# InternRobotics/InternNav

Measured on AMD Instinct MI355X. Metric: policy steps/sec/node, higher is better.
Workload: dtype bf16

## Files before the change

include/internnav_amd.h:

```cpp
#ifndef INTERNNAV_AMD_H
#define INTERNNAV_AMD_H

#include <stddef.h>
#include <stdint.h>

#ifdef __cplusplus
extern "C" {
#endif

#define INA_ABI_VERSION 8

#define INA_ACT_NONE_C 0
#define INA_ACT_GELU_ERF_C 1
#define INA_ACT_GELU_TANH_C 2
#define INA_ACT_RELU_C 3
#define INA_ACT_SILU_C 4
#define INA_ACT_MISH_C 5
#define INA_BF16 0
#define INA_F32 1

int ina_abi_version(void);
const char* ina_last_error(void);
int ina_device_check(char* name, int n);
int ina_struct_size(int k);
int ina_set_workspace_slot(int slot);
int ina_workspace_retired(void);
int ina_prof_enable(int on);
int ina_prof_read(int kind, double* ms_total, int64_t* launches, double* flops, double* bytes);
int ina_prof_read_sub(int kind, int sub, double* ms_total, int64_t* launches, double* flops, double* bytes);

typedef struct ina_gemm_args {
    const void* A;
    const void* W;
    void* C;
    const float* bias;
    const float* colscale;
    const float* rowscale;
    const void* R;
    int32_t M, N, K;
    int32_t lda, ldw, ldc, ldr;
    int32_t act;
    int32_t out_dtype;
    int32_t res_dtype;
    int32_t glu;
    int32_t rowscale_div;
    int32_t batch;
    int64_t strideA, strideW, strideC, strideR;
    int32_t force_cfg;
    int32_t group_m;
    const float* norm_gamma;
    float norm_eps;
    int32_t a_dtype;
    float* seg_stats;
    float seg_eps;
    int32_t _pad_seg;
    const void* Wp;
} ina_gemm_args;
int ina_gemm_bf16(const ina_gemm_args* args, void* stream);
int ina_gemm_w8(const ina_gemm_args* args, const void* W8, const int8_t* wexp, void* stream);
int ina_gemm_preshuffle(const void* W, void* Wp, int32_t N, int32_t K, int64_t ldw, void* stream);
int ina_gemm_select(const ina_gemm_args* args, int* kernel);

typedef struct ina_attn_args {
    const void* Q;
    const void* K;
    const void* V;
    void* O;
    int64_t q_bs, q_rs, q_hs;
    int64_t k_bs, k_rs, k_hs;
    int64_t v_bs, v_rs, v_hs;
    int64_t o_bs, o_rs, o_hs;
    int32_t B, H, Hkv;
    int32_t Lq, Lk;
    int32_t D;
    int32_t causal;
    int32_t kv_start;
    int32_t kv_bdiv;
    float scale;
    const int32_t* cu_q;
    const int32_t* cu_k;
    const float* head_gate;
    const int32_t* k_len;
    int32_t accumulate;
    uint32_t drop_seed;
    uint32_t drop_thresh;
    float drop_scale;
    int32_t kernel;
    int32_t _pad0;
    const uint32_t* drop_salt;
    const float* rope_cos;
    const float* rope_sin;
    const void* k_new;
    const void* v_new;
    int64_t kn_bs, kn_rs, kn_hs;
// ... 388 lines not shown
```

internnav_amd/_lib.py:

```python
from __future__ import annotations

import ctypes as C
from pathlib import Path

_HERE = Path(__file__).resolve().parent
LIB_PATH = _HERE / "libinternnav_amd.so"

c_void_p, c_int32, c_int64, c_float = C.c_void_p, C.c_int32, C.c_int64, C.c_float


class GemmArgs(C.Structure):
    _fields_ = [
        ("A", c_void_p), ("W", c_void_p), ("C", c_void_p),
        ("bias", c_void_p), ("colscale", c_void_p), ("rowscale", c_void_p), ("R", c_void_p),
        ("M", c_int32), ("N", c_int32), ("K", c_int32),
        ("lda", c_int32), ("ldw", c_int32), ("ldc", c_int32), ("ldr", c_int32),
        ("act", c_int32), ("out_dtype", c_int32), ("res_dtype", c_int32), ("glu", c_int32),
        ("rowscale_div", c_int32), ("batch", c_int32),
        ("strideA", c_int64), ("strideW", c_int64), ("strideC", c_int64), ("strideR", c_int64),
        ("force_cfg", c_int32), ("group_m", c_int32),
        ("norm_gamma", c_void_p), ("norm_eps", c_float), ("a_dtype", c_int32),
        ("seg_stats", c_void_p), ("seg_eps", c_float), ("_pad_seg", c_int32),
        ("Wp", c_void_p),
    ]


class AttnArgs(C.Structure):
    _fields_ = [
        ("Q", c_void_p), ("K", c_void_p), ("V", c_void_p), ("O", c_void_p),
        ("q_bs", c_int64), ("q_rs", c_int64), ("q_hs", c_int64),
        ("k_bs", c_int64), ("k_rs", c_int64), ("k_hs", c_int64),
        ("v_bs", c_int64), ("v_rs", c_int64), ("v_hs", c_int64),
        ("o_bs", c_int64), ("o_rs", c_int64), ("o_hs", c_int64),
        ("B", c_int32), ("H", c_int32), ("Hkv", c_int32),
        ("Lq", c_int32), ("Lk", c_int32), ("D", c_int32),
        ("causal", c_int32), ("kv_start", c_int32), ("kv_bdiv", c_int32),
        ("scale", c_float),
        ("cu_q", c_void_p), ("cu_k", c_void_p), ("head_gate", c_void_p), ("k_len", c_void_p),
        ("accumulate", c_int32), ("drop_seed", C.c_uint32), ("drop_thresh", C.c_uint32), ("drop_scale", c_float),
        ("kernel", c_int32), ("_pad0", c_int32), ("drop_salt", c_void_p),
        ("rope_cos", c_void_p), ("rope_sin", c_void_p), ("k_new", c_void_p), ("v_new", c_void_p),
        ("kn_bs", c_int64), ("kn_rs", c_int64), ("kn_hs", c_int64),
    ]


class RowMap(C.Structure):
    _fields_ = [("seg_len", c_int32), ("seg_stride", c_int32), ("off", c_int32), ("_pad", c_int32)]


class NormArgs(C.Structure):
    _fields_ = [
        ("X", c_void_p), ("Y", c_void_p), ("Y32", c_void_p),
        ("gamma", c_void_p), ("beta", c_void_p), ("mod_scale", c_void_p), ("gate", c_void_p), ("G", c_void_p), ("P", c_void_p),
        ("in_map", RowMap), ("out_map", RowMap),
        ("rows", c_int32), ("C", c_int32),
# ... 187 lines not shown
                ("lddp", c_int32), ("loss_scale", c_float)]


class AdamwArgs(C.Structure):
    _fields_ = [("p", c_void_p), ("g", c_void_p), ("m", c_void_p), ("v", c_void_p), ("p_bf16", c_void_p), ("sumsq_parts", c_void_p),
                ("norm_out", c_void_p), ("n", c_int64), ("n_parts", c_int32), ("zero_grad", c_int32),
                ("lr", c_float), ("beta1", c_float), ("beta2", c_float), ("eps", c_float), ("wd", c_float), ("bc1", c_float), ("bc2", c_float),
                ("max_norm", c_float), ("grad_scale", c_float), ("_pad", c_int32)]


class GemmDwArgs(C.Structure):
    _fields_ = [("DY", c_void_p), ("X", c_void_p), ("dW", c_void_p), ("db", c_void_p), ("partial", c_void_p), ("partial_elems", c_int64),
                ("rows", c_int32), ("N", c_int32), ("K", c_int32), ("dy_dt", c_int32), ("lddy", c_int32), ("ldx", c_int32), ("ldw", c_int32), ("splits", c_int32)]


class GemmNnArgs(C.Structure):
    _fields_ = [("X", c_void_p), ("W", c_void_p), ("partial", c_void_p), ("partial_elems", c_int64),
                ("M", c_int32), ("N", c_int32), ("K", c_int32), ("ldx", c_int32), ("ldw", c_int32), ("splits", c_int32)]


class AttnBwdArgs(C.Structure):
    _fields_ = [("f", AttnArgs), ("dO", c_void_p), ("dQ", c_void_p), ("dK", c_void_p), ("dV", c_void_p), ("lse", c_void_p), ("delta", c_void_p),
                ("dq_bs", c_int64), ("dq_rs", c_int64), ("dq_hs", c_int64), ("dkv_bs", c_int64), ("dkv_rs", c_int64), ("dkv_hs", c_int64),
                ("kv_row0", c_int32), ("nsplit", c_int32), ("part", c_void_p), ("dq32", c_void_p), ("stage", c_int32), ("_pad", c_int32)]


SYMBOLS = {
    "ina_abi_version": (C.c_int, []),
    "ina_last_error": (C.c_char_p, []),
    "ina_device_check": (C.c_int, [C.c_char_p, C.c_int]),
    "ina_gemm_bf16": (C.c_int, [C.POINTER(GemmArgs), c_void_p]),
    "ina_gemm_w8": (C.c_int, [C.POINTER(GemmArgs), c_void_p, c_void_p, c_void_p]),
    "ina_gemm_select": (C.c_int, [C.POINTER(GemmArgs), C.POINTER(C.c_int)]),
    "ina_gemm_preshuffle": (C.c_int, [c_void_p, c_void_p, c_int32, c_int32, c_int64, c_void_p]),
    "ina_attention_bf16": (C.c_int, [C.POINTER(AttnArgs), c_void_p]),
    "ina_norm_bf16": (C.c_int, [C.POINTER(NormArgs), c_void_p]),
    "ina_patchify": (C.c_int, [C.POINTER(PatchifyArgs), c_void_p]),
    "ina_embed3": (C.c_int, [C.POINTER(Embed3Args), c_void_p]),
    "ina_goal_slots": (C.c_int, [c_void_p, c_int32, c_int32, c_int32, c_int32, c_int32, c_void_p, c_int32, c_int32, c_void_p, c_void_p, c_void_p,
                                 c_void_p, c_int32, c_void_p, c_void_p, c_void_p, c_int32, c_void_p, c_void_p, c_void_p, c_int32, c_void_p,
                                 c_void_p, c_int32, c_int32, c_void_p]),
    "ina_kv_copy": (C.c_int, [c_int32, c_void_p, c_int32, c_void_p, c_int32, c_int64, c_int64, c_int64, c_void_p]),
    "ina_attention_prefix": (C.c_int, [c_void_p, c_int64, c_int64, c_int64, c_void_p, c_int64, c_int64, c_int64, c_void_p, c_void_p, c_int64, c_int64,
                                       c_int64, c_int32, c_void_p, c_void_p, c_int64, c_int64, c_int64, c_void_p, c_void_p, c_void_p, c_int32, c_int32,
                                       c_int32, c_int32, c_int32, c_int32, c_float, c_void_p]),
    "ina_memory_gather": (C.c_int, [c_void_p, c_int64, c_void_p, c_void_p, c_void_p, c_void_p, c_void_p, c_void_p, c_void_p, c_int32, c_int32, c_int32,
                                    c_int32, c_int32, c_int32, c_int32, c_void_p]),
    "ina_traj_actions": (C.c_int, [c_void_p, c_int32, c_int32, c_int32, c_int32, c_void_p, c_int32, c_void_p, c_void_p, c_int32, c_void_p]),
    "ina_head3": (C.c_int, [C.POINTER(Head3Args), c_void_p]),
    "ina_seqpool_head": (C.c_int, [C.POINTER(SeqpoolArgs), c_void_p]),
    "ina_select_traj": (C.c_int, [C.POINTER(SelectArgs), c_void_p]),
    "ina_pool_act": (C.c_int, [C.POINTER(PoolActArgs), c_void_p]),
    "ina_gather_rows": (C.c_int, [C.POINTER(GatherArgs), c_void_p]),
    "ina_rope_bf16": (C.c_int, [C.POINTER(RopeArgs), c_void_p]),
    "ina_mrope_table": (C.c_int, [C.POINTER(MropeTableArgs), c_void_p]),
    "ina_argmax_rows": (C.c_int, [C.POINTER(ArgmaxArgs), c_void_p]),
    "ina_token_seen_set": (C.c_int, [c_void_p, c_int32, c_void_p, c_int32, c_void_p, c_int32, c_int32, c_void_p]),
    "ina_argmax_penalty_rows": (C.c_int, [c_void_p, c_int32, c_int32, c_int32, c_void_p, c_int32, C.c_float, c_int32, c_void_p, c_void_p]),
    "ina_logprob_rows": (C.c_int, [c_void_p, c_int32, c_int32, c_int32, c_void_p, c_int32, C.c_float, c_int32, c_void_p, c_void_p, c_void_p, c_void_p,
                                   c_void_p]),
    "ina_dit_attention": (C.c_int, [C.POINTER(DitAttnArgs), c_void_p]),
    "ina_resize_u8": (C.c_int, [C.POINTER(ResizeU8Args), c_void_p]),
    "ina_qwen_patchify_u8": (C.c_int, [C.POINTER(QwenPatchifyArgs), c_void_p]),
    "ina_u8_lut": (C.c_int, [C.POINTER(U8LutArgs), c_void_p]),
    "ina_resize_f32": (C.c_int, [C.POINTER(ResizeF32Args), c_void_p]),
    "ina_dit_rowchain": (C.c_int, [C.POINTER(DitRowchainArgs), c_void_p]),
# ... 54 lines not shown
```

internnav_amd/csrc/abi.cpp:

```cpp
#include <stdarg.h>
#include <stdio.h>
#include <string.h>
#include <cmath>

#include "common.h"
#include "kernels.h"

static thread_local char g_err[1024] = "";

void ina_set_error(const char* fmt, ...) {
    va_list ap;
    va_start(ap, fmt);
    vsnprintf(g_err, sizeof(g_err), fmt, ap);
    va_end(ap);
}

#include <mutex>
#include <vector>
namespace {
struct ProfRec { int kind, sub; hipEvent_t a, b; double flops, bytes; };
thread_local int g_prof_sub = 0;
bool g_prof_on = false;
std::vector<ProfRec> g_prof;
std::mutex g_prof_mu;
// ... 167 lines not shown
}

int ina_traj_actions(void* traj, int32_t traj_dtype, int32_t B, int32_t S, int32_t T, int32_t* actions, int32_t max_actions, int32_t* count,
                     double* traj_out, int32_t scale_in_place, void* stream) {
    return ina_launch_traj_actions(traj, traj_dtype, B, S, T, actions, max_actions, count, traj_out, scale_in_place, reinterpret_cast<hipStream_t>(stream));
}

int ina_token_seen_set(uint32_t* seen, int32_t ld_words, const int32_t* ids, int32_t ld_ids, const int32_t* lens, int32_t rows, int32_t n, void* stream) {
    return ina_launch_token_seen_set(seen, ld_words, ids, ld_ids, lens, rows, n, reinterpret_cast<hipStream_t>(stream));
}

int ina_argmax_penalty_rows(const float* X, int32_t ldx, int32_t rows, int32_t n, uint32_t* seen, int32_t ld_words, float penalty, int32_t mark,
                            int32_t* out, void* stream) {
    return ina_launch_argmax_penalty(X, ldx, rows, n, seen, ld_words, penalty, mark, out, reinterpret_cast<hipStream_t>(stream));
}

int ina_logprob_rows(const float* X, int32_t ldx, int32_t rows, int32_t n, uint32_t* seen, int32_t ld_words, float penalty, int32_t mark,
                     const int32_t* target, int32_t* tok, float* logprob, float* margin, void* stream) {
    INA_REQUIRE(X && tok && logprob, "logprob_rows: X, tok and logprob required");
    INA_REQUIRE(rows >= 0 && n >= 1 && ldx >= n, "logprob_rows: bad arguments rows=%d n=%d ldx=%d (rows >= 0, n >= 1, ldx >= n)", rows, n, ldx);
    if (seen) {
        INA_REQUIRE((long)ld_words * 32 >= (long)n, "logprob_rows: ld_words=%d holds fewer than n=%d bits", ld_words, n);
        INA_REQUIRE(std::isfinite(penalty) && penalty > 0.f, "logprob_rows: repetition penalty %g is not a strictly positive finite float", (double)penalty);
    }
    INA_REQUIRE(!mark || (seen && !target), "logprob_rows: mark needs a seen set and is refused with a target (teacher forcing selects nothing)");
    if (rows == 0) return 0;
    return ina_launch_logprob(X, ldx, rows, n, seen, ld_words, penalty, mark, target, tok, logprob, margin, reinterpret_cast<hipStream_t>(stream));
}

int ina_gemm_select(const ina_gemm_args* args, int* kernel) {
    INA_REQUIRE(args != nullptr && kernel != nullptr, "gemm_select: null argument");
    GemmArgs p;
    return ina_plan_gemm(*args, p, *kernel);
}

int ina_attention_bf16(const ina_attn_args* args, void* stream) {
    INA_REQUIRE(args != nullptr, "attention: null args");
    return ina_launch_attention(*args, reinterpret_cast<hipStream_t>(stream));
}

int ina_norm_bf16(const ina_norm_args* args, void* stream) {
    INA_REQUIRE(args != nullptr, "norm: null args");
    return ina_launch_norm(*args, reinterpret_cast<hipStream_t>(stream));
}

int ina_struct_size(int k) {
    switch (k) {
        case 0: return (int)sizeof(ina_gemm_args);
        case 1: return (int)sizeof(ina_attn_args);
        case 2: return (int)sizeof(ina_norm_args);
        case 3: return (int)sizeof(ina_patchify_args);
        case 4: return (int)sizeof(ina_embed3_args);
        case 5: return (int)sizeof(ina_head3_args);
        case 6: return (int)sizeof(ina_seqpool_args);
        case 7: return (int)sizeof(ina_select_args);
        case 8: return (int)sizeof(ina_pool_act_args);
        case 9: return (int)sizeof(ina_gather_args);
        case 10: return (int)sizeof(ina_rope_args);
        case 11: return (int)sizeof(ina_mrope_table_args);
        case 12: return (int)sizeof(ina_argmax_args);
        case 13: return (int)sizeof(ina_dit_attn_args);
        case 14: return (int)sizeof(ina_resize_u8_args);
        case 15: return (int)sizeof(ina_qwen_patchify_args);
        case 16: return (int)sizeof(ina_u8_lut_args);
        case 17: return (int)sizeof(ina_resize_f32_args);
        case 18: return (int)sizeof(ina_gn_mish_args);
// ... 57 lines not shown
```

internnav_amd/csrc/gemm.hip:

```cpp
#include "common.h"
#include "kernels.h"
#include "gemm_epilogue.h"

namespace {

template <int BM, int BN, int BK, int WM, int WN>
struct GemmCfg {
    static constexpr int NT = WM * WN * 64;
    static constexpr int TM = BM / WM;
    static constexpr int TN = BN / WN;
    static constexpr int FM = TM / 16;
    static constexpr int FN = TN / 16;
    static constexpr int LDS_K = BK + 8;
    static constexpr int CPR = BK / 8;
    static constexpr int A_CHUNKS = BM * CPR / NT;
    static constexpr int B_CHUNKS = BN * CPR / NT;
    static constexpr size_t LDS_BYTES = size_t(2) * (BM + BN) * LDS_K * sizeof(bf16);
};

template <int BM, int BN, int BK, int WM, int WN>
__global__ __launch_bounds__(WM* WN * 64) void gemm_bf16_nt_kernel(GemmArgs p) {
    using C = GemmCfg<BM, BN, BK, WM, WN>;
    extern __shared__ __attribute__((aligned(16))) char smem_raw[];
    bf16* As = reinterpret_cast<bf16*>(smem_raw);
// ... 174 lines not shown
                const long slots = 256L * wg_per_cu;
                const double rounds = shared ? (double)tiles / slots : (double)((tiles + slots - 1) / slots);
                return rounds * wg_per_cu * (bm / 128.0) * (bn / 128.0) / rate;
            };
            const double c11 = cost(128, 128, 2, 0.85), c14 = cost(256, 128, 1, 0.92), c18 = cost(256, 256, 1, 1.18);
            const double c21 = cost(192, 256, 1, 0.97);
            cfg = (c18 < c14 && c18 < c11) ? 18 : (c14 < c11 ? 14 : 11);
            const double best = cfg == 18 ? c18 : cfg == 14 ? c14 : c11;
            if (c21 < best) cfg = 21;
            if (cfg == 18 && p.R && p.out_dtype == INA_DT_F32 && p.K <= 4096) cfg = 33;
            if (cfg == 18 && !p.R && p.K >= 2048 && p.K <= 4096 && p.N >= 4096 && p.M >= 2048 && ina_gemm_w4_contract(p)) cfg = 39;
            if ((cfg == 39 || (cfg == 18 && p.K >= 8192 && ina_gemm_w4_contract(p))) && p.Wp && p.N % 16 == 0 && p.batch == 1) cfg = 40;
        }
    }
    {
        static const int known[] = {1, 2, 3, 4, 5, 11, 14, 18, 21, 22, 26, 27, 33, 34, 35, 39, 40};
        bool ok = false;
        for (int k : known) ok = ok || k == cfg;
        INA_REQUIRE(ok, "gemm: unknown tile config %d", cfg);
    }
    if (cfg == 40) INA_REQUIRE(p.Wp && p.N % 16 == 0 && p.batch == 1, "gemm: tile config 40 needs the fragment-ordered copy of W (Wp), N %% 16 == 0, no batch (N=%d)", p.N);
    if (cfg == 39 || cfg == 40)
        INA_REQUIRE(ina_gemm_w4_contract(p), "gemm: tile configs 39 / 40 (four-wave 256 x 256 tile) need K %% 64 == 0, 16-byte aligned output / residual rows "
                    "and act none .. silu (M=%d N=%d K=%d ldc=%d act=%d)", p.M, p.N, p.K, p.ldc, p.act);
    INA_REQUIRE(!p.seg_stats || cfg == 34 || cfg == 35, "gemm: seg_stats (LayerNorm statistics of the produced rows) exist in the row-panel kernels only "
                "(K = 384, plain epilogue, M >= 16384): this call would run tile config %d (M=%d N=%d K=%d)", cfg, p.M, p.N, p.K);
    if (cfg == 34 || cfg == 35)
        INA_REQUIRE(ina_gemm_rowpanel_contract(p), "gemm: tile configs 34 / 35 (row-panel kernels) need K = 384, N %% 128 == 0, M %% 32 == 0, bf16 output, "
                    "no scales / residual, bias + activation or SiLU-GLU (M=%d N=%d K=%d)", p.M, p.N, p.K);
    kernel = cfg;
    return 0;
}

int ina_launch_gemm(const GemmArgs& p_in, hipStream_t stream) {
    GemmArgs p;
    int cfg = 0;
    if (int rc = ina_plan_gemm(p_in, p, cfg)) return rc;
    if (cfg == 30) return ina_launch_gemm_skinny_prenorm(p, stream);
    if (cfg == 32) return ina_launch_gemm_skinny_fused(p, stream);
    ina_prof_set_sub(cfg);
    switch (cfg) {
        case 1: return launch_cfg<128, 128, 64, 2, 2>(p, stream);
        case 2: return launch_cfg<64, 128, 64, 2, 2>(p, stream);
        case 3: return launch_cfg<64, 128, 64, 1, 4>(p, stream);
        case 4: return launch_cfg<64, 64, 64, 2, 2>(p, stream);
        case 5: return launch_cfg<128, 64, 64, 2, 2>(p, stream);
        case 11: case 14: case 18: case 21: case 22: case 26: case 27: case 33: case 39: case 40: return ina_launch_gemm_glds(p, stream, cfg);
        case 34: case 35: return ina_launch_gemm_rowpanel(p, stream, cfg);
        default: ina_set_error("gemm: unknown tile config %d", cfg); return -2;
    }
}
```

internnav_amd/csrc/kernels.h:

```cpp
#pragma once
#include <hip/hip_runtime.h>
#include <stddef.h>
#include <stdint.h>

#include "../../include/internnav_amd.h"

using GemmArgs = ina_gemm_args;
using AttnArgs = ina_attn_args;
using NormArgs = ina_norm_args;
using PatchifyArgs = ina_patchify_args;
using Embed3Args = ina_embed3_args;
using Head3Args = ina_head3_args;
using SeqpoolArgs = ina_seqpool_args;
using SelectArgs = ina_select_args;
using PoolActArgs = ina_pool_act_args;
using GatherArgs = ina_gather_args;
using RopeArgs = ina_rope_args;
using MropeTableArgs = ina_mrope_table_args;
using ArgmaxArgs = ina_argmax_args;
using DitAttnArgs = ina_dit_attn_args;
using ResizeU8Args = ina_resize_u8_args;
using QwenPatchifyArgs = ina_qwen_patchify_args;
using U8LutArgs = ina_u8_lut_args;
using ResizeF32Args = ina_resize_f32_args;
using DitRowchainArgs = ina_dit_rowchain_args;
using GnMishArgs = ina_gn_mish_args;
using PadRowsArgs = ina_pad_rows_args;
using DdimStepArgs = ina_ddim_step_args;
using EwArgs = ina_ew_args;
using ColsumArgs = ina_colsum_args;
using NormBwdArgs = ina_norm_bwd_args;
using TransposeArgs = ina_transpose_args;
using SparseRowsArgs = ina_sparse_rows_args;
using SmallLinearArgs = ina_small_linear_args;
using MseArgs = ina_mse_args;
using AdamwArgs = ina_adamw_args;
using GemmNnArgs = ina_gemm_nn_args;
using AttnBwdArgs = ina_attn_bwd_args;

int ina_launch_gemm(const GemmArgs& p, hipStream_t stream);
int ina_plan_gemm(const GemmArgs& p_in, GemmArgs& p, int& kernel);
int ina_launch_gemm_skinny_prenorm(const GemmArgs& p, hipStream_t stream);
int ina_launch_gemm_glds(const GemmArgs& p, hipStream_t stream, int cfg);
int ina_launch_gemm_skinny_fused(const GemmArgs& p, hipStream_t stream);
int ina_launch_gemm_w8(const GemmArgs& p, const void* W8, const int8_t* wexp, hipStream_t stream);
int ina_launch_gemm_rowpanel(const GemmArgs& p, hipStream_t stream, int cfg);
bool ina_gemm_rowpanel_contract(const GemmArgs& p);
bool ina_gemm_w4_contract(const GemmArgs& p);
int ina_launch_gemm_preshuffle(const void* W, void* Wp, int N, int K, long ldw, hipStream_t stream);
int ina_launch_gemm_w4(const GemmArgs& p, hipStream_t stream, int cfg);
int ina_launch_attention(const AttnArgs& p, hipStream_t stream);
bool ina_attention_wide_eligible(const AttnArgs& p);
bool ina_attention_wide_contract(const AttnArgs& p);
int ina_launch_attention_wide(const AttnArgs& p, hipStream_t stream);
int ina_launch_norm(const NormArgs& p, hipStream_t stream);
int ina_launch_patchify(const PatchifyArgs& p, hipStream_t stream);
int ina_launch_embed3(const Embed3Args& p, hipStream_t stream);
int ina_launch_goal_slots(void* Y, int ldy, int y_dtype, int L, int slot0, int nslots, const float* P, int B, int D, const int32_t* kind,
                          const int32_t* row, float* embed, const float* point, int n_point, const float* point_w, const float* point_b,
                          const float* image_tok, int n_image, const float* image_w, const float* image_b, const float* pixel_tok,
                          int n_pixel, const float* pixel_w, const float* pixel_b, int ntok, int E, hipStream_t stream);
int ina_launch_kv_copy(int to_engine, const int64_t* layer_base, int n_layers, const int64_t* seq, int n_seq, long engine_rows, long row_bytes,
                       long max_rows, hipStream_t stream);
int ina_launch_attention_prefix(const void* Q, long q_ps, long q_rs, long q_hs, void* O, long o_ps, long o_rs, long o_hs, const void* Kc,
                                const void* Vc, long c_ss, long c_rs, long c_hs, int n_slots, const void* Ks, const void* Vs, long s_ps, long s_rs,
                                long s_hs, const int32_t* slot, const int32_t* pfx_len, const int32_t* suf_len, int P, int m, int H, int Hkv, int D,
                                int max_pfx, float scale, hipStream_t stream);
int ina_launch_memory_gather(void* out, long out_env_stride, float* ring, const float* fresh, const float* blank, const float* pe,
                             const int32_t* env, const int32_t* head, const int32_t* count, int n, int max_envs, int M, int ntok, int C, int depth,
                             int stride, hipStream_t stream);
int ina_launch_traj_actions(void* traj, int traj_dtype, int B, int S, int T, int32_t* actions, int max_actions, int32_t* count, double* traj_out,
                            int scale_in_place, hipStream_t stream);
int ina_launch_token_seen_set(uint32_t* seen, int ld_words, const int32_t* ids, int ld_ids, const int32_t* lens, int rows, int n,
                              hipStream_t stream);
// ... 33 lines not shown
```

internnav_amd/ops.py:

```python
from __future__ import annotations

import contextlib
import ctypes as C
from typing import Optional

import torch

from . import _lib
from ._lib import AttnArgs, GemmArgs, NormArgs

ACT = {None: 0, "none": 0, "gelu": 1, "gelu_erf": 1, "gelu_tanh": 2, "relu": 3, "silu": 4, "mish": 5, "tanh": 6}
_DT = {torch.bfloat16: 0, torch.float32: 1}


_AUTO_CFG = 0


@contextlib.contextmanager
def shared_tail():
    global _AUTO_CFG
    keep, _AUTO_CFG = _AUTO_CFG, -1
    try:
        yield
    finally:
        _AUTO_CFG = keep


def _stream() -> int:
    return torch.cuda.current_stream().cuda_stream


def _ptr(t: Optional[torch.Tensor]) -> Optional[int]:
    return None if t is None else t.data_ptr()


def _f32(t: Optional[torch.Tensor]) -> Optional[torch.Tensor]:
    if t is None:
        return None
    assert t.dtype == torch.float32 and t.is_contiguous(), "f32 parameter vectors must be contiguous float32"
    return t


def _as2d(x: torch.Tensor) -> torch.Tensor:
    assert x.stride(-1) == 1, "last dimension must be contiguous"
    if x.dim() == 2:
        return x
    return x.reshape(-1, x.shape[-1]) if x.is_contiguous() else x


def linear(x: torch.Tensor, w: torch.Tensor, bias: Optional[torch.Tensor] = None, act=None,
           colscale: Optional[torch.Tensor] = None, residual: Optional[torch.Tensor] = None,
           out: Optional[torch.Tensor] = None, out_dtype=torch.bfloat16, glu: bool = False,
           rowscale: Optional[torch.Tensor] = None, rowscale_div: int = 1, force_cfg: int = 0,
           batched: bool = False, group_m: int = 0, prenorm=None, w_frag: Optional[torch.Tensor] = None, seg_stats=None) -> torch.Tensor:
    assert (x.dtype == torch.bfloat16 or prenorm is not None) and w.dtype == torch.bfloat16
    assert w.dim() == 2 and w.stride(1) == 1
    N, K = w.shape
    n_out = N // 2 if glu else N
    a = GemmArgs()
    if batched:
        assert x.dim() == 3 and x.stride(2) == 1 and out is not None and out.dim() == 3 and out.stride(2) == 1
        Bt, M, _ = x.shape
        assert out.shape == (Bt, M, n_out)
        a.A, a.C = x.data_ptr(), out.data_ptr()
        a.lda, a.ldc = x.stride(1), out.stride(1)
        a.batch, a.strideA, a.strideC = Bt, x.stride(0), out.stride(0)
        if residual is not None:
            assert residual.stride(-1) == 1 and residual.shape[-2:] == (M, n_out)
            a.R, a.ldr, a.res_dtype = residual.data_ptr(), residual.stride(-2), _DT[residual.dtype]
            a.strideR = residual.stride(0) if residual.dim() == 3 else 0
    else:
        lead = x.shape[:-1]
        x2 = _as2d(x)
        assert x2.dim() == 2
        M = x2.shape[0]
        if out is None:
            out = torch.empty(*lead, n_out, dtype=out_dtype, device=x.device)
        o2 = _as2d(out)
        assert o2.shape == (M, n_out), f"out {tuple(o2.shape)} vs {(M, n_out)}"
        a.A, a.C = x2.data_ptr(), o2.data_ptr()
        a.lda, a.ldc = x2.stride(0), o2.stride(0)
        a.batch = 1
        if residual is not None:
            r2 = _as2d(residual)
            assert r2.shape == (M, n_out)
            a.R, a.ldr, a.res_dtype = r2.data_ptr(), r2.stride(0), _DT[r2.dtype]
    assert x.shape[-1] == K, f"K mismatch {tuple(w.shape)} vs {tuple(x.shape)}"
    a.W, a.ldw = w.data_ptr(), w.stride(0)
    a.bias, a.colscale, a.rowscale = _ptr(_f32(bias)), _ptr(_f32(colscale)), _ptr(_f32(rowscale))
    a.M, a.N, a.K = M, N, K
    a.act = ACT[act] if not isinstance(act, int) else act
    a.out_dtype = _DT[out.dtype]
    a.glu = 1 if glu else 0
    a.rowscale_div = rowscale_div
    a.force_cfg = force_cfg if force_cfg else _AUTO_CFG
    a.group_m = group_m
    if seg_stats is not None:
        st, se = seg_stats
        assert not batched and st.dtype == torch.float32 and st.is_contiguous() and st.numel() >= M * (N // 384) * 2 and N % 384 == 0
        a.seg_stats, a.seg_eps = st.data_ptr(), float(se)
    if w_frag is not None:
        assert w_frag.dtype == torch.bfloat16 and w_frag.is_contiguous() and w_frag.numel() == N * K and N % 16 == 0 and K % 32 == 0
        a.Wp = w_frag.data_ptr()
    if prenorm is not None:
        gamma, eps = prenorm
        assert not batched and x.dtype in (torch.bfloat16, torch.float32) and gamma.dtype == torch.float32 and gamma.is_contiguous() and gamma.numel() == K
        a.norm_gamma, a.norm_eps, a.a_dtype = gamma.data_ptr(), float(eps), _DT[x.dtype]
    _lib.check(_lib.lib().ina_gemm_bf16(C.byref(a), _stream()), "gemm_bf16")
    return out


def gemm_preshuffle(w: torch.Tensor, out: Optional[torch.Tensor] = None) -> torch.Tensor:
    assert w.dtype == torch.bfloat16 and w.dim() == 2 and w.stride(1) == 1
    N, K = w.shape
    if out is None:
        out = torch.empty(N * K, dtype=torch.bfloat16, device=w.device)
    assert out.dtype == torch.bfloat16 and out.is_contiguous() and out.numel() == N * K
    _lib.check(_lib.lib().ina_gemm_preshuffle(w.data_ptr(), out.data_ptr(), N, K, w.stride(0), _stream()), "gemm_preshuffle")
    return out


W8_MAX = 448.0
W8_EXP_RANGE = 64


def w8_pack(q: torch.Tensor) -> torch.Tensor:
    assert q.dtype == torch.uint8 and q.dim() == 2 and q.shape[1] % 128 == 0, "w8 layout: uint8 [N, K] with K % 128 == 0"
    N, K = q.shape
    return q.reshape(N, K // 128, 4, 4, 8).transpose(2, 3).reshape(N, K).contiguous()
# ... 645 lines not shown
```

internnav_amd/qwen_vl.py:

```python
from __future__ import annotations

import weakref
from typing import Dict, List, Optional, Sequence, Tuple

import numpy as np
import torch

from . import ops
from .runtime import CapacityError


def vision_window_permutation(grids: Sequence[Tuple[int, int, int]], merge: int = 2, window: int = 112, patch: int = 14):
    win = window // merge // patch
    idx_all, cu, base = [], [0], 0
    for t, h, w in grids:
        gh, gw = h // merge, w // merge
        idx = np.arange(t * gh * gw).reshape(t, gh, gw)
        ph, pw = win - gh % win, win - gw % win
        nh, nw = (gh + ph) // win, (gw + pw) // win
        pad = np.pad(idx, ((0, 0), (0, ph), (0, pw)), constant_values=-100)
        pad = pad.reshape(t, nh, win, nw, win).transpose(0, 1, 3, 2, 4).reshape(t, nh * nw, win * win)
        lens = (pad != -100).sum(-1).reshape(-1)
        flat = pad.reshape(-1)
        idx_all.append(flat[flat != -100] + base)
# ... 155 lines not shown
        if self._engine is not None and self.is_view:
            self._engine.materialize_kv([(self, b) for b in range(len(self)) if self._views[b] is not None])
        return self

    def __deepcopy__(self, memo):
        kv = [None if t is None else t.clone() for t in self.kv]
        c = EngineKVCache([None if t is None else t.clone() for t in self.token_ids], kv, self._engine, list(self._views))
        c.materialize()
        return c


W8_DECODER_KEYS = ("self_attn.q_proj.weight", "self_attn.k_proj.weight", "self_attn.v_proj.weight", "self_attn.o_proj.weight",
                   "mlp.gate_proj.weight", "mlp.up_proj.weight", "mlp.down_proj.weight")


def w8_roundtrip_state_dict(sd, cfg: dict) -> dict:
    names = {f"model.layers.{i}.{k}" for i in range(cfg["t_layers"]) for k in W8_DECODER_KEYS} | {"lm_head.weight"}
    out = {}
    for k in sd.keys():
        v = sd[k]
        out[k] = ops.w8_quantize(v.to(torch.bfloat16).contiguous())[2].to(v.dtype) if k in names else v
    return out


def _interleave16(a: torch.Tensor, b: torch.Tensor) -> torch.Tensor:
    n, k = a.shape
    return torch.stack([a.view(n // 16, 16, k), b.view(n // 16, 16, k)], dim=1).reshape(2 * n, k).contiguous()


def _pad_rows(t: torch.Tensor, n: int) -> torch.Tensor:
    return t if t.shape[0] == n else torch.cat([t, t.new_zeros((n - t.shape[0],) + tuple(t.shape[1:]))], 0)


class QwenVLEngine:

    def __init__(self, weights, cfg: dict, device="cuda:0", max_seqs: int = 16, max_seq_len: int = 1024, max_patches: int = 16 * 3136,
                 frag_weights: Optional[bool] = None, w8_decode: bool = False, token_logprobs: bool = False, max_decode: int = 128):
        dev = torch.device(device)
        bf, f32 = torch.bfloat16, torch.float32
        self.cfg, self.device = cfg, dev
        self.B_max, self.S_max, self.Np_max = max_seqs, max_seq_len, max_patches
        self.fuse_decode_norm = True
        self.split_prefill = True
        self.split_serial = False
        self._side = None
        self.fuse_decode_rope = True
        self.tap = None
        D, I = cfg["v_hidden"], cfg["v_inter"]
        Ip = (I + 63) // 64 * 64
        self.vD, self.vI, self.vH, self.vhd = D, Ip, cfg["v_heads"], D // cfg["v_heads"]
        H, TI = cfg["t_hidden"], cfg["t_inter"]
        self.H, self.TI, self.nh, self.nkv = H, TI, cfg["t_heads"], cfg["t_kv_heads"]
        self.hd = H // self.nh
        self.qkv_w = (self.nh + 2 * self.nkv) * self.hd
        self.kv_w = 2 * self.nkv * self.hd
        W = weights

        def w(k):
            return W[k].to(device=dev, dtype=bf).contiguous()

        def f(k):
            return W[k].to(device=dev, dtype=f32).contiguous()

        self.v_patch = W["visual.patch_embed.proj.weight"].to(device=dev, dtype=bf).reshape(D, -1).contiguous()
        self.v_blocks = []
        for i in range(cfg["v_depth"]):
            b = f"visual.blocks.{i}."
            gw_, uw = _pad_rows(W[b + "mlp.gate_proj.weight"].to(dev).float(), Ip), _pad_rows(W[b + "mlp.up_proj.weight"].to(dev).float(), Ip)
            gb, ub = _pad_rows(W[b + "mlp.gate_proj.bias"].to(dev).float(), Ip), _pad_rows(W[b + "mlp.up_proj.bias"].to(dev).float(), Ip)
            dw = W[b + "mlp.down_proj.weight"].to(dev).float()
            dw = torch.cat([dw, dw.new_zeros(D, Ip - I)], 1) if Ip != I else dw
            self.v_blocks.append(dict(
                n1=f(b + "norm1.weight"), n2=f(b + "norm2.weight"), qkv_w=w(b + "attn.qkv.weight"), qkv_b=f(b + "attn.qkv.bias"),
                proj_w=w(b + "attn.proj.weight"), proj_b=f(b + "attn.proj.bias"),
                gu_w=_interleave16(gw_, uw).to(bf), gu_b=_interleave16(gb[:, None], ub[:, None]).reshape(-1).contiguous(),
                down_w=dw.to(bf).contiguous(), down_b=f(b + "mlp.down_proj.bias"), full=i in cfg["v_fullatt"]))
        self.m_ln = f("visual.merger.ln_q.weight")
# ... 386 lines not shown
        P.pop("_split_info", None)
        if int(pl.max()) != 0:
            pos_run = np.zeros((3, B, Sr), dtype=np.int64)
            for b in range(B):
                n = S - pl[b]
                pos_run[:, b, :n] = pos3[:, b, pl[b]:]
                pos_run[:, b, n:] = pos3[:, b, -1:]
            uniform = bool((pl == pl[0]).all())
            P["prefill"] = self._phase(B, Sr, pos_run, pl, k_len=None if uniform else pl + Sr)
        nxt = pos3[:, :, -1].max(axis=0) + 1
        P["next_pos"] = nxt
        P["decode"] = [self._phase(B, 1, (nxt + j)[None, :, None], S + j) for j in range(max(n_decode - 1, 0))]
        if with_latents:
            nq = self.latent_q.shape[0]
            cur = S + max(n_decode - 1, 0)
            m = 1 if n_decode > 0 else 0
            p = (nxt + (cur - S))[None, :, None] + np.arange(m + nq)[None, None, :]
            P["latents"] = self._phase(B, m + nq, p, cur)
            P["lat_m"] = m
        return P

    def run_prefill(self, P: dict, pixel_values: Optional[torch.Tensor]):
        if self._kv_views:
            self._kv_evict({b: int(w) for b, w in enumerate(P["prefill"]["w0"])})
        ops.gather_rows(self.embed, self.x_in, src=P["ids"])
        if self.split_prefill and P.get("split") and self.tap is None:
            if "traj_src" in P:
                ops.gather_rows(self.latent_q, self.x_in, src=P["traj_src"], dst=P["traj_dst"])
            main = torch.cuda.current_stream()
            if self._side is None:
                self._side = torch.cuda.Stream(device=self.device)
            self._side.wait_stream(main)

            def half(s):
                vp = s["vision"]
                emb = self.run_vision(vp, pixel_values[vp["p0"]: vp["p0"] + vp["Np"]])
                tok = self.emb_tok[s["tok0"]: s["tok0"] + s["n_tok"]]
                ops.gather_rows(emb, tok, src=s["img_src"])
                ops.gather_rows(tok, self.x_in, dst=s["img_dst"])
                self._layers(s["prefill"])

            with ops.shared_tail():
                if self.split_serial:
                    half(P["split"][1])
                else:
                    with torch.cuda.stream(self._side):
                        half(P["split"][1])
                half(P["split"][0])
            main.wait_stream(self._side)
            return
        if P["vision"] is not None:
            emb = self.run_vision(P["vision"], pixel_values)
            n = P["img_src"].shape[0]
            ops.gather_rows(emb, self.emb_tok[:n], src=P["img_src"])
            ops.gather_rows(self.emb_tok[:n], self.x_in, dst=P["img_dst"])
        for c, dst in P["cached"]:
            ops.gather_rows(c, self.x_in, dst=dst)
        if "traj_src" in P:
            ops.gather_rows(self.latent_q, self.x_in, src=P["traj_src"], dst=P["traj_dst"])
        self._layers(P["prefill"])

    def fresh_image_embeds(self, P: dict) -> Dict[int, torch.Tensor]:
        return {k: self.emb_tok[a:b].clone() for k, a, b in P["fresh_tokens"]}

    def run_decode(self, P: dict, tokens_out: torch.Tensor, j0: int = 0, j1: Optional[int] = None):
        B, S, n = P["B"], P["S_run"], P["n_decode"]
        j1 = n if j1 is None else min(j1, n)
        if n == 0 or j0 >= j1:
            return
        pen = P.get("rep_penalty")
        if j0 == 0:
            if pen is not None:
                self._seen_init(P)
            self._last_logits(B, S, S - 1, penalty=pen, col=0)
        for j in range(j0, j1):
            tokens_out[:, j].copy_(self.next_tok[:B])
            if j == n - 1:
                break
            ops.gather_rows(self.embed, self.x_in, src=self.next_tok[:B], rows=B)
            self._layers(P["decode"][j])
            self._last_logits(B, 1, 0, penalty=pen, col=j + 1)

# ... 231 lines not shown
```

Measured before the change: 302.7.

## Split GEMM row tail into a smaller-tile second launch to reduce wave quantization

Adds a cost model over tile families and CU count that predicts when the last partial wave of 256x256 tiles leaves most CUs idle. In that case it launches the GEMM as a 256-row-aligned body plus a tail using a 128-tile config. It also rewrites config 21 calls to a 256-tile config when the model predicts a saving. Inside shared_tail the split is disabled, and an optional joint-decoder path runs the prefill layers once after both vision halves instead of per half. The change adds an extra launch per split GEMM and relies on hand-set throughput constants.

```diff
diff --git a/include/internnav_amd.h b/include/internnav_amd.h
--- a/include/internnav_amd.h
+++ b/include/internnav_amd.h
@@ -53,13 +53,14 @@
     int32_t a_dtype;
     float* seg_stats;
     float seg_eps;
-    int32_t _pad_seg;
+    int32_t tail_split;
     const void* Wp;
 } ina_gemm_args;
 int ina_gemm_bf16(const ina_gemm_args* args, void* stream);
 int ina_gemm_w8(const ina_gemm_args* args, const void* W8, const int8_t* wexp, void* stream);
 int ina_gemm_preshuffle(const void* W, void* Wp, int32_t N, int32_t K, int64_t ldw, void* stream);
 int ina_gemm_select(const ina_gemm_args* args, int* kernel);
+int ina_gemm_tail_split(const ina_gemm_args* args, int32_t cus, int* kernel, int* row_tile, int* tail_kernel, double* us_whole, double* us_split);
 
 typedef struct ina_attn_args {
     const void* Q;
diff --git a/internnav_amd/_lib.py b/internnav_amd/_lib.py
--- a/internnav_amd/_lib.py
+++ b/internnav_amd/_lib.py
@@ -20,7 +20,7 @@
         ("strideA", c_int64), ("strideW", c_int64), ("strideC", c_int64), ("strideR", c_int64),
         ("force_cfg", c_int32), ("group_m", c_int32),
         ("norm_gamma", c_void_p), ("norm_eps", c_float), ("a_dtype", c_int32),
-        ("seg_stats", c_void_p), ("seg_eps", c_float), ("_pad_seg", c_int32),
+        ("seg_stats", c_void_p), ("seg_eps", c_float), ("tail_split", c_int32),
         ("Wp", c_void_p),
     ]
 
@@ -274,6 +274,8 @@
     "ina_gemm_bf16": (C.c_int, [C.POINTER(GemmArgs), c_void_p]),
     "ina_gemm_w8": (C.c_int, [C.POINTER(GemmArgs), c_void_p, c_void_p, c_void_p]),
     "ina_gemm_select": (C.c_int, [C.POINTER(GemmArgs), C.POINTER(C.c_int)]),
+    "ina_gemm_tail_split": (C.c_int, [C.POINTER(GemmArgs), C.c_int32, C.POINTER(C.c_int), C.POINTER(C.c_int), C.POINTER(C.c_int),
+                                      C.POINTER(C.c_double), C.POINTER(C.c_double)]),
     "ina_gemm_preshuffle": (C.c_int, [c_void_p, c_void_p, c_int32, c_int32, c_int64, c_void_p]),
     "ina_attention_bf16": (C.c_int, [C.POINTER(AttnArgs), c_void_p]),
     "ina_norm_bf16": (C.c_int, [C.POINTER(NormArgs), c_void_p]),
diff --git a/internnav_amd/csrc/abi.cpp b/internnav_amd/csrc/abi.cpp
--- a/internnav_amd/csrc/abi.cpp
+++ b/internnav_amd/csrc/abi.cpp
@@ -223,6 +223,19 @@
     INA_REQUIRE(args != nullptr && kernel != nullptr, "gemm_select: null argument");
     GemmArgs p;
     return ina_plan_gemm(*args, p, *kernel);
+}
+
+int ina_gemm_tail_split(const ina_gemm_args* args, int32_t cus, int* kernel, int* row_tile, int* tail_kernel, double* us_whole, double* us_split) {
+    INA_REQUIRE(args != nullptr && kernel != nullptr && row_tile != nullptr && tail_kernel != nullptr, "gemm_tail_split: null argument");
+    GemmArgs p;
+    *row_tile = *tail_kernel = 0;
+    if (int rc = ina_plan_gemm(*args, p, *kernel)) return rc;
+    double whole = 0.0, split = 0.0;
+    if (*kernel != 30 && *kernel != 32)
+        if (int rc = ina_plan_gemm_tail(p, *kernel, cus > 0 ? cus : 256, *row_tile, *tail_kernel, whole, split)) return rc;
+    if (us_whole) *us_whole = whole;
+    if (us_split) *us_split = split;
+    return 0;
 }
 
 int ina_attention_bf16(const ina_attn_args* args, void* stream) {
diff --git a/internnav_amd/csrc/gemm.hip b/internnav_amd/csrc/gemm.hip
--- a/internnav_amd/csrc/gemm.hip
+++ b/internnav_amd/csrc/gemm.hip
@@ -230,12 +230,85 @@
     return 0;
 }
 
-int ina_launch_gemm(const GemmArgs& p_in, hipStream_t stream) {
-    GemmArgs p;
-    int cfg = 0;
-    if (int rc = ina_plan_gemm(p_in, p, cfg)) return rc;
-    if (cfg == 30) return ina_launch_gemm_skinny_prenorm(p, stream);
-    if (cfg == 32) return ina_launch_gemm_skinny_fused(p, stream);
+namespace {
+struct TileFamily { int cfg, bm, bn, wg; double tflops; };
+constexpr TileFamily kFamilies[] = {{40, 256, 256, 1, 1300.0}, {39, 256, 256, 1, 1250.0}, {18, 256, 256, 1, 1220.0}, {33, 256, 256, 1, 1120.0},
+                                    {11, 128, 128, 2, 940.0},  {14, 256, 128, 1, 950.0},  {21, 192, 256, 1, 1000.0}};
+constexpr double kAlone = 1.5, kLaunchUs = 6.0, kMinGain = 0.08;
+
+const TileFamily* family(int cfg) {
+    for (const TileFamily& f : kFamilies)
+        if (f.cfg == cfg) return &f;
+    return nullptr;
+}
+double family_us(const TileFamily& f, long rows, long N, long K, int cus) {
+    const long tiles = ((rows + f.bm - 1) / f.bm) * ((N + f.bn - 1) / f.bn), slots = (long)cus * f.wg;
+    const double tile_us = 2.0 * f.bm * f.bn * K * cus / (f.tflops * 1e6);
+    const long rem = tiles % slots;
+    double us = (double)(tiles / slots) * f.wg * tile_us;
+    if (rem) us += rem <= cus ? tile_us * (f.wg > 1 ? f.wg / kAlone : 1.0) : f.wg * tile_us;
+    return us;
+}
+}
+
+int ina_plan_gemm_tail(const GemmArgs& p, int& cfg, int cus, int& row_tile, int& tail_cfg, double& us_whole, double& us_split) {
+    row_tile = 0;
+    tail_cfg = 0;
+    us_whole = us_split = 0.0;
+    const int ts = p.tail_split;
+    if (cfg == 21 && ts == 0 && p.force_cfg == 0) {
+        GemmArgs q = p, planned;
+        q.force_cfg = -1;
+        int alt = 0, rt = 0, tc = 0;
+        double w = 0.0, sp = 0.0;
+        if (ina_plan_gemm(q, planned, alt) != 0 || alt == 21) return 0;
+        if (int rc = ina_plan_gemm_tail(planned, alt, cus, rt, tc, w, sp)) return rc;
+        us_whole = family_us(*family(21), p.M, p.N, p.K, cus);
+        us_split = sp;
+        if (rt > 0 && sp < (1.0 - kMinGain) * us_whole) cfg = alt, row_tile = rt, tail_cfg = tc;
+        return 0;
+    }
+    const TileFamily* big = family(cfg);
+    if (big && big->bm != 256) big = nullptr;
+    if (ts == 1 || (ts == 0 && !big)) return 0;
+    INA_REQUIRE(big, "gemm: tail_split=%d needs one of the 256 x 256 tile configs (18, 33, 39, 40); this call runs config %d", ts, cfg);
+    INA_REQUIRE(cus > 0, "gemm: tail split over %d CUs", cus);
+    const int tm = (p.M + 255) / 256, tn = (p.N + 255) / 256;
+    const bool rows_ok = p.batch == 1 && !p.seg_stats && (!p.rowscale || 256 % p.rowscale_div == 0);
+    auto tail_family = [&](long rows, double& us) {
+        const TileFamily* best = nullptr;
+        for (int c : {11, 14}) {
+            const TileFamily* f = family(c);
+            const double t = family_us(*f, rows, p.N, p.K, cus);
+            if (!best || t < us) best = f, us = t;
+        }
+        return best->cfg;
+    };
+    if (ts != 0) {
+        const long n = ts < 0 ? -(long)ts : ts;
+        INA_REQUIRE(n >= 1 && n < tm, "gemm: tail_split=%d: row tile %ld is outside the %d row tiles of M=%d (a body and a tail need 1 .. %d)", ts, n, tm, p.M, tm - 1);
+        INA_REQUIRE(rows_ok, "gemm: a forced tail split needs batch 1, no seg_stats and rowscale_div dividing 256 (batch=%d rowscale_div=%d)", p.batch, p.rowscale_div);
+        double us;
+        row_tile = (int)n;
+        tail_cfg = tail_family(p.M - n * 256, us);
+        return 0;
+    }
+    if (!rows_ok || p.M <= 64) return 0;
+    const long tiles = (long)tm * tn, rem = tiles % cus;
+    const long b = tiles / cus * cus / tn;
+    if (tiles < cus || rem == 0 || 2 * rem >= cus || b < 1 || b >= tm) return 0;
+    us_whole = family_us(*big, p.M, p.N, p.K, cus);
+    double us_tail;
+    const int tc = tail_family(p.M - b * 256, us_tail);
+    us_split = family_us(*big, b * 256, p.N, p.K, cus) + us_tail + kLaunchUs;
+    if (us_split < (1.0 - kMinGain) * us_whole) {
+        row_tile = (int)b;
+        tail_cfg = tc;
+    }
+    return 0;
+}
+
+static int launch_tiled(const GemmArgs& p, hipStream_t stream, int cfg) {
     ina_prof_set_sub(cfg);
     switch (cfg) {
         case 1: return launch_cfg<128, 128, 64, 2, 2>(p, stream);
@@ -248,3 +321,28 @@
         default: ina_set_error("gemm: unknown tile config %d", cfg); return -2;
     }
 }
+
+int ina_launch_gemm(const GemmArgs& p_in, hipStream_t stream) {
+    GemmArgs p;
+    int cfg = 0;
+    if (int rc = ina_plan_gemm(p_in, p, cfg)) return rc;
+    if (cfg == 30) return ina_launch_gemm_skinny_prenorm(p, stream);
+    if (cfg == 32) return ina_launch_gemm_skinny_fused(p, stream);
+    int row_tile = 0, tail_cfg = 0;
+    double us_whole, us_split;
+    if (int rc = ina_plan_gemm_tail(p, cfg, 256, row_tile, tail_cfg, us_whole, us_split)) return rc;
+    if (row_tile == 0) return launch_tiled(p, stream, cfg);
+    const long r0 = (long)row_tile * 256;
+    const size_t oes = p.out_dtype == INA_DT_BF16 ? 2 : 4, res = p.res_dtype == INA_DT_BF16 ? 2 : 4;
+    GemmArgs body = p, tail = p;
+    body.M = (int)r0;
+    tail.M = p.M - (int)r0;
+    tail.A = reinterpret_cast<const char*>(p.A) + (size_t)r0 * p.lda * sizeof(bf16);
+    tail.C = reinterpret_cast<char*>(p.C) + (size_t)r0 * p.ldc * oes;
+    if (p.R) tail.R = reinterpret_cast<const char*>(p.R) + (size_t)r0 * p.ldr * res;
+    if (p.rowscale) tail.rowscale = p.rowscale + r0 / p.rowscale_div;
+    tail.Wp = nullptr;
+    tail.group_m = 0;
+    if (int rc = launch_tiled(body, stream, cfg)) return rc;
+    return launch_tiled(tail, stream, tail_cfg);
+}
diff --git a/internnav_amd/csrc/kernels.h b/internnav_amd/csrc/kernels.h
--- a/internnav_amd/csrc/kernels.h
+++ b/internnav_amd/csrc/kernels.h
@@ -40,6 +40,7 @@
 
 int ina_launch_gemm(const GemmArgs& p, hipStream_t stream);
 int ina_plan_gemm(const GemmArgs& p_in, GemmArgs& p, int& kernel);
+int ina_plan_gemm_tail(const GemmArgs& p, int& cfg, int cus, int& row_tile, int& tail_cfg, double& us_whole, double& us_split);
 int ina_launch_gemm_skinny_prenorm(const GemmArgs& p, hipStream_t stream);
 int ina_launch_gemm_glds(const GemmArgs& p, hipStream_t stream, int cfg);
 int ina_launch_gemm_skinny_fused(const GemmArgs& p, hipStream_t stream);
diff --git a/internnav_amd/ops.py b/internnav_amd/ops.py
--- a/internnav_amd/ops.py
+++ b/internnav_amd/ops.py
@@ -18,12 +18,25 @@
 
 @contextlib.contextmanager
 def shared_tail():
-    global _AUTO_CFG
-    keep, _AUTO_CFG = _AUTO_CFG, -1
+    global _AUTO_CFG, _TAIL_SPLIT
+    keep, _AUTO_CFG, _TAIL_SPLIT = (_AUTO_CFG, _TAIL_SPLIT), -1, 1
     try:
         yield
     finally:
-        _AUTO_CFG = keep
+        _AUTO_CFG, _TAIL_SPLIT = keep
+
+
+_TAIL_SPLIT = 0
+
+
+@contextlib.contextmanager
+def no_tail_split():
+    global _TAIL_SPLIT
+    keep, _TAIL_SPLIT = _TAIL_SPLIT, 1
+    try:
+        yield
+    finally:
+        _TAIL_SPLIT = keep
 
 
 def _stream() -> int:
@@ -52,7 +65,7 @@
            colscale: Optional[torch.Tensor] = None, residual: Optional[torch.Tensor] = None,
            out: Optional[torch.Tensor] = None, out_dtype=torch.bfloat16, glu: bool = False,
            rowscale: Optional[torch.Tensor] = None, rowscale_div: int = 1, force_cfg: int = 0,
-           batched: bool = False, group_m: int = 0, prenorm=None, w_frag: Optional[torch.Tensor] = None, seg_stats=None) -> torch.Tensor:
+           batched: bool = False, group_m: int = 0, prenorm=None, w_frag: Optional[torch.Tensor] = None, seg_stats=None, tail_split: int = 0) -> torch.Tensor:
     assert (x.dtype == torch.bfloat16 or prenorm is not None) and w.dtype == torch.bfloat16
     assert w.dim() == 2 and w.stride(1) == 1
     N, K = w.shape
@@ -95,6 +108,7 @@
     a.rowscale_div = rowscale_div
     a.force_cfg = force_cfg if force_cfg else _AUTO_CFG
     a.group_m = group_m
+    a.tail_split = tail_split if tail_split else _TAIL_SPLIT
     if seg_stats is not None:
         st, se = seg_stats
         assert not batched and st.dtype == torch.float32 and st.is_contiguous() and st.numel() >= M * (N // 384) * 2 and N % 384 == 0
diff --git a/internnav_amd/qwen_vl.py b/internnav_amd/qwen_vl.py
--- a/internnav_amd/qwen_vl.py
+++ b/internnav_amd/qwen_vl.py
@@ -211,6 +211,9 @@
     return t if t.shape[0] == n else torch.cat([t, t.new_zeros((n - t.shape[0],) + tuple(t.shape[1:]))], 0)
 
 
+JOINT_DECODER_SEQS = frozenset()
+
+
 class QwenVLEngine:
 
     def __init__(self, weights, cfg: dict, device="cuda:0", max_seqs: int = 16, max_seq_len: int = 1024, max_patches: int = 16 * 3136,
@@ -222,6 +225,7 @@
         self.fuse_decode_norm = True
         self.split_prefill = True
         self.split_serial = False
+        self.joint_decoder = None
         self._side = None
         self.fuse_decode_rope = True
         self.tap = None
@@ -674,13 +678,16 @@
                 self._side = torch.cuda.Stream(device=self.device)
             self._side.wait_stream(main)
 
+            joint = P["B"] in JOINT_DECODER_SEQS if self.joint_decoder is None else bool(self.joint_decoder)
+
             def half(s):
                 vp = s["vision"]
                 emb = self.run_vision(vp, pixel_values[vp["p0"]: vp["p0"] + vp["Np"]])
                 tok = self.emb_tok[s["tok0"]: s["tok0"] + s["n_tok"]]
                 ops.gather_rows(emb, tok, src=s["img_src"])
                 ops.gather_rows(tok, self.x_in, dst=s["img_dst"])
-                self._layers(s["prefill"])
+                if not joint:
+                    self._layers(s["prefill"])
 
             with ops.shared_tail():
                 if self.split_serial:
@@ -690,6 +697,8 @@
                         half(P["split"][1])
                 half(P["split"][0])
             main.wait_stream(self._side)
+            if joint:
+                self._layers(P["prefill"])
             return
         if P["vision"] is not None:
             emb = self.run_vision(P["vision"], pixel_values)
```

Result: no change. 302.9, median of 5 (+0.1%).
